# xu-ji/IIC

Measured on AMD Instinct MI355X. Metric: paired-images/sec, STL10 96x96 ClusterNet5g+IID_loss, higher is better.
Workload: dtype bf16; 1 GPU; STL10 96x96 ClusterNet5g IID+ (cluster_sobel.py train step), batch 660 pairs/GPU, 5 sub-heads, k=70, bf16 MFMA convs / fp32 stem+heads+loss, fused HIP Adam; global_batch_pairs=660, input=96x96x1 grey -> sobel 2ch, parallelism=dp1, streams=2, launch=hip-graph replay: 6 linear graph segments, the two views on two streams

## Files before the change

iic_amd/csrc/common.h:

```cpp
#pragma once
#include <hip/hip_runtime.h>
#include <stdint.h>

#include <atomic>
#include <mutex>
#include <utility>

#define IIC_OK 0
#define IIC_ERR_ARG (-1)
#define IIC_ERR_LAUNCH (-2)
#define IIC_ERR_UNSUPPORTED (-3)

#ifdef IIC_DEBUG_HOOKS
#define IIC_HOOK extern "C" __attribute__((visibility("default")))
#define IIC_SWITCH(var, dflt, setter) \
  static int var = dflt;              \
  IIC_HOOK void setter(int v) { var = v; }
IIC_HOOK int iic_debug_get_ablate(void);
#else
#define IIC_SWITCH(var, dflt, setter) static constexpr int var = dflt;
static inline constexpr int iic_debug_get_ablate(void) { return 0; }
#endif

typedef __attribute__((ext_vector_type(8))) __bf16 bf16x8;
typedef __attribute__((ext_vector_type(4))) short s16x4;
typedef __attribute__((ext_vector_type(16))) float f32x16;
typedef __attribute__((ext_vector_type(4))) float f32x4;
typedef __attribute__((ext_vector_type(4))) unsigned int u32x4;
typedef __attribute__((ext_vector_type(2))) unsigned int u32x2;

typedef uint16_t bf16_t;

static inline int iic_launch_status() {
  hipError_t e = hipGetLastError();
  return e == hipSuccess ? IIC_OK : IIC_ERR_LAUNCH;
}

static constexpr long IIC_LDS_BYTES = 160 * 1024;

template <auto Kernel, typename... Args>
inline int iic_launch_lds(dim3 grid, dim3 block, size_t lds, hipStream_t s, Args&&... args) {
  static std::atomic<size_t> limit{48 * 1024};
  if (lds > limit.load(std::memory_order_acquire)) {
    static std::mutex raise;
// ... 128 lines not shown
```

iic_amd/csrc/conv_igemm_bd.hip:

```cpp
#include "common.h"
#include "conv_tile.h"
#include "../../include/iic_hip.h"

__device__ __forceinline__ void bd_bload(u32x4& d, const unsigned char* p) {
  asm volatile("global_load_dwordx4 %0, %1, off" : "=v"(d) : "v"(p) : "memory");
}
template <int N>
__device__ __forceinline__ void bd_bwait(u32x4& d) {
  asm volatile("s_waitcnt vmcnt(%1)" : "+v"(d) : "i"(N) : "memory");
}

struct bd_blk {
  int bw, bh, nbx, nby;
  int PW, npix, mul;
};

#define BD_BM 256
#define BD_BN 128
#define BD_THREADS 256
#define BD_PROF_SLOTS 16
#ifndef BD_STORE_UB
#define BD_STORE_UB 8
#endif

template <bool GATHER, int ABL, int MS, int RED, int WN = 2>
__device__ __forceinline__ void bd_tile(
    const iic_conv_geom& g, const bf16_t* __restrict__ in, const unsigned char* __restrict__ wfrag,
    bf16_t* __restrict__ out, float* __restrict__ stats, const bf16_t* __restrict__ res_grad,
    const bf16_t* __restrict__ res_act, int accumulate, int lds_a_bytes,
    const bf16_t* __restrict__ red_y, const float* __restrict__ red_coef,
    const bf16_t* __restrict__ red_y2, float* __restrict__ red_stats, float* __restrict__ red_stats2,
    unsigned long long* __restrict__ prof, int blk_in_class, int nwg_class, const bd_blk& B) {
  constexpr int BNT = WN * 64, NWM = 4 / WN;
  constexpr bool CANBLK = !GATHER && MS * 32 * (4 / WN) == 256;
  const bool blk = CANBLK && B.bw > 0;
  constexpr int CLD = BNT + 8;
  constexpr bool PROF = (ABL & 128) != 0;
  constexpr bool NEWORD = (ABL & 256) == 0;
  constexpr bool SWZ = (ABL & 512) == 0;
  unsigned long long t_stamp[8];
  unsigned long long t_bsum = 0, t_b0 = 0;
  int t_nb = 0;
  if (PROF) t_stamp[0] = __builtin_readcyclecounter();
  constexpr int BM = MS * 32 * NWM, WR = MS * 32;
  extern __shared__ __attribute__((aligned(16))) unsigned char smem_raw[];
  unsigned char* sA = smem_raw;
  int* s_pin = reinterpret_cast<int*>(smem_raw + lds_a_bytes);
  int* s_pout = s_pin + BM;
  float* s_red = reinterpret_cast<float*>(s_pout + BM);
  unsigned char* s_key = reinterpret_cast<unsigned char*>(s_red + NWM * 2 * BNT);
  bf16_t* sC = reinterpret_cast<bf16_t*>(smem_raw);

  const int tid = threadIdx.x, lane = tid & 63;
  const int wave = __builtin_amdgcn_readfirstlane(tid >> 6);
  const int wm = WN == 2 ? wave >> 1 : wave, wn = WN == 2 ? wave & 1 : 0;
  const int l31 = lane & 31, g5 = lane >> 5;

  const int nt = g.Cout / BNT;
  const int tix = xcd_tile_index(blk_in_class, nwg_class);
  const int mtile = tix / nt, ntile = tix - mtile * nt;
  const int n0 = ntile * BNT;
  const int m0 = mtile * BM;
// ... 22 lines not shown
    }
  } else if (tid < BM) {
    int pin, pout;
    igemm_row_pixels(g, m0 + tid, pin, pout);
    s_pin[tid] = pin;
    s_pout[tid] = pout;
  }
  __syncthreads();
  const int p_lo = blk ? 0 : s_pin[0];
  const int npix = GATHER ? BM : (blk ? B.npix : (BM >= 192 ? g.NP256 : g.NP));
  const int keyw = blk ? B.PW : g.in_Wp;
  const int jskip = blk ? B.PW - B.bw
                        : ((!GATHER && g.sx == 1 && ((g.in_Wp - g.MX) & 1) == 0) ? g.in_Wp - g.MX : 0);
  auto dense_of = [&](int p) { return p - jskip * (p / keyw); };
  int arow[MS];
  int drow[MS];
#pragma unroll
  for (int ms = 0; ms < MS; ++ms) {
    const int row = wm * WR + ms * 32 + l31;
    const int pr = GATHER ? row : (s_pin[row] - p_lo);
    arow[ms] = SWZ ? pr : pr * ROWB + g5 * 16;
    drow[ms] = (SWZ && !GATHER) ? dense_of(s_pin[row]) : pr;
  }
  if (!GATHER && jskip != 0) {
    for (int r = tid; r < npix; r += BD_THREADS) s_key[r] = (unsigned char)((dense_of(p_lo + r) >> 1) & 7);
    __syncthreads();
  }
  const int v_tapd = v_tapoff - jskip * (v_tapoff / keyw);
  const int nblk = (npix * 128 + 1023) >> 10;
  auto dma_patch = [&](int c0) {
    for (int kb = wave; kb < nblk; kb += BD_THREADS / 64) {
      const int q = kb * 64 + lane;
      const int r = q >> 3;
      const int ls = (q & 7) ^ (GATHER ? ((r >> 1) & 7)
                                       : (jskip != 0 ? (int)s_key[r < npix ? r : npix - 1]
                                                     : (((p_lo + r) >> 1) & 7)));
      long p = GATHER ? (long)s_pin[r < BM ? r : BM - 1] : (long)p_lo + r;
      if (blk) {
        const int rc = r < npix ? r : npix - 1;
        const int py = (rc * B.mul) >> 16;
        p = (long)blk_glo + py * g.in_Wp + (rc - py * B.PW);
      }
      p = p < in_pixels ? p : in_pixels - 1;
      __builtin_amdgcn_global_load_lds(
          (const __attribute__((address_space(1))) void*)(in + (p * g.Cin + c0 + ls * 8)),
          (__attribute__((address_space(3))) void*)(sA + kb * 1024), 16, 0, 0);
    }
    asm volatile("s_waitcnt vmcnt(0)" ::: "memory");
  };
  auto a_base = [&](int R, int D) { return R * 128 + (((g5 ^ (D >> 1)) & 1) << 4); };
  auto a_kk = [&](int D) { return ((D >> 2) & 3) << 5; };

  f32x16 acc[MS][2];
// ... 208 lines not shown
      }
  __syncthreads();
  if (PROF) t_stamp[4] = __builtin_readcyclecounter();
  TileRed tr;
  if (RED) tile_red_zero(tr);
  if (!(ABL & 32))
    igemm_store_tile<BNT, BM, BD_THREADS, 8, RED, (BM == 256 ? BD_STORE_UB : 4)>(sC, s_pout, out, res_grad, res_act, accumulate,
                                                                 g.Cout, n0, tid, red_y, red_coef, red_y2, &tr);
  if (RED)
    igemm_red_finish<BNT, BD_THREADS, RED>(tr, reinterpret_cast<float*>(smem_raw), red_stats, red_stats2,
                                             g.Cout, n0, tid);
  if (PROF && prof && tid == 0) {
    unsigned long long* q = prof + (long)blockIdx.x * BD_PROF_SLOTS;
    const unsigned long long t_end = __builtin_readcyclecounter();
    q[0] = t_stamp[0]; q[1] = t_stamp[1]; q[2] = t_stamp[2]; q[3] = t_stamp[3]; q[4] = t_stamp[4];
    q[5] = t_end; q[6] = t_bsum; q[7] = (unsigned long long)t_nb;
    q[8] = (unsigned long long)__builtin_amdgcn_s_getreg((32 - 1) << 11 | 0 << 6 | 4)
           | ((unsigned long long)__builtin_amdgcn_s_getreg((4 - 1) << 11 | 0 << 6 | 20) << 32);
    q[9] = (unsigned long long)tix;
    q[10] = __builtin_amdgcn_s_memrealtime();
  }
}

template <bool GATHER, int ABL, int MS, int RED, int WN = 2>
__global__ __launch_bounds__(BD_THREADS, ((MS == 4 || WN == 1) ? 2 : 3)) void conv_igemm_bd_kernel(
    const iic_conv_geom g, const bf16_t* __restrict__ in, const unsigned char* __restrict__ wfrag,
    bf16_t* __restrict__ out, float* __restrict__ stats, const bf16_t* __restrict__ res_grad,
    const bf16_t* __restrict__ res_act, int accumulate, int num_mtiles, int lds_a_bytes,
    const bf16_t* __restrict__ red_y, const float* __restrict__ red_coef,
    const bf16_t* __restrict__ red_y2, float* __restrict__ red_stats, float* __restrict__ red_stats2,
    unsigned long long* __restrict__ prof, const bd_blk B) {
  bd_tile<GATHER, ABL, MS, RED, WN>(g, in, wfrag, out, stats, res_grad, res_act, accumulate, lds_a_bytes, red_y,
                                    red_coef, red_y2, red_stats, red_stats2, prof, (int)blockIdx.x,
                                    num_mtiles * (g.Cout / (WN * 64)), B);
}

__global__ void weight_prep_frag_kernel(const float* __restrict__ w, bf16_t* __restrict__ o, int Co,
                                        int Ci, int T, int mode) {
  const int Nn = mode ? Ci : Co, Kk = mode ? Co : Ci;
  const int n32 = Nn >> 5, nchunks = Kk >> 6;
  const long total = (long)T * Co * Ci;
  for (long i = (long)blockIdx.x * blockDim.x + threadIdx.x; i < total;
       i += (long)gridDim.x * blockDim.x) {
    const int e = (int)(i & 7), lane = (int)((i >> 3) & 63), ks = (int)((i >> 9) & 3);
    long r = i >> 11;
    const int j = (int)(r % n32);
    r /= n32;
    const int kc = (int)(r % nchunks), t = (int)(r / nchunks);
    const int n = j * 32 + (lane & 31), k = kc * 64 + ks * 16 + (lane >> 5) * 8 + e;
    const int co = mode ? k : n, ci = mode ? n : k;
    o[i] = f32_to_bf16(w[((long)co * Ci + ci) * T + t]);
  }
}

int iic_p64_supported(const iic_conv_geom* g);
int iic_p64_launch(const iic_conv_geom* g, const void* in, const void* wfrag, void* out, float* stats,
                   const void* res_grad, const void* res_act, int accumulate, const void* red_y,
                   const float* red_coef, const void* red_y2, float* red_stats, float* red_stats2,
                   void* stream);
int iic_pw_supported(const iic_conv_geom* g);
int iic_pw_launch(const iic_conv_geom* g, const void* in, const void* wfrag, void* out, float* stats,
                  const void* res_grad, const void* res_act, int accumulate, const void* red_y,
                  const float* red_coef, const void* red_y2, float* red_stats, float* red_stats2, void* stream);
IIC_SWITCH(g_p64_enabled, 1, iic_debug_enable_p64)
IIC_SWITCH(g_p64_red, 0, iic_debug_p64_red)

extern "C" {

#ifdef IIC_DEBUG_HOOKS
static unsigned long long* g_bd_prof = nullptr;
IIC_HOOK void iic_debug_bd_prof(void* buf) { g_bd_prof = (unsigned long long*)buf; }
IIC_HOOK int iic_debug_bd_prof_slots(void) { return BD_PROF_SLOTS; }
#else
static constexpr unsigned long long* g_bd_prof = nullptr;
#endif

static long bd_lds_a(const iic_conv_geom* g, int ms, int wn = 2) {
  const long bm = ms * 32 * (4 / wn);
  const long npix = g->ntaps == 1 ? bm : (bm >= 192 ? g->NP256 : g->NP);
  long a = (npix * 128 + 1023) & ~1023L;
  long c = bm * (wn * 64 + 8) * 2;
  long m = a > c ? a : c;
  return (m + 15) & ~15L;
}

static long bd_key_bytes(const iic_conv_geom* g, int ms, int wn = 2) {
  const int jskip = (g->ntaps > 1 && g->sx == 1 && ((g->in_Wp - g->MX) & 1) == 0) ? g->in_Wp - g->MX : 0;
  return jskip != 0 ? (((long)(ms * 32 * (4 / wn) >= 192 ? g->NP256 : g->NP) + 15) & ~15L) : 0;
}
static long bd_lds_total(const iic_conv_geom* g, int ms, int wn = 2) {
  return bd_lds_a(g, ms, wn) + 2L * ms * 32 * (4 / wn) * 4 + 4L * BD_BN * 4 + bd_key_bytes(g, ms, wn);
}
IIC_SWITCH(g_bd_w1, 1, iic_debug_bd_w1)
static bool bd_w1_ok(const iic_conv_geom* g) {
  return g_bd_w1 && g->Cout % 64 == 0 && g->Cout % BD_BN != 0 && g->ntaps > 1 && g->NP256 > 0 &&
         bd_lds_total(g, 2, 1) <= IIC_LDS_BYTES;
}
IIC_SWITCH(g_bd_ms, 0, iic_debug_bd_ms)
static int bd_pick_ms(const iic_conv_geom* g) {
  const bool ok4 = (g->ntaps == 1 || g->NP256 > 0) && bd_lds_total(g, 4) <= IIC_LDS_BYTES;
  const bool ok2 = (g->ntaps == 1 || g->NP > 0) && bd_lds_total(g, 2) <= IIC_LDS_BYTES;
  if (g_bd_ms == 4) return ok4 ? 4 : (ok2 ? 2 : 0);
  if (g_bd_ms == 2) return ok2 ? 2 : (ok4 ? 4 : 0);
  if (ok4 && ok2 && g->ntaps > 1) {
    const long M = igemm_rows_host(g);
    if (((M + 255) / 256) * (g->Cout / BD_BN) * 2 <= 512) return 2;
  }
  return ok4 ? 4 : (ok2 ? 2 : 0);
}

static int bd_block_config(const iic_conv_geom* g, bd_blk* B, int wn);
int iic_conv_igemm_frag_supported(const iic_conv_geom* g) {
  if (!g) return 0;
  if (g_p64_enabled && iic_p64_supported(g)) return 1;
// ... 93 lines not shown
      const long a = ((long)B1.npix * 128 + 1023) & ~1023L, c = (long)BD_BM * (64 + 8) * 2;
      la1 = (int)(((a > c ? a : c) + 15) & ~15L);
      lds1 = la1 + 2L * BD_BM * 4 + 4L * BD_BN * 4 + ((B1.npix + 15) & ~15L);
    }
    hipStream_t s1 = (hipStream_t)stream;
    int rc1 = IIC_OK;
#define BD_LAUNCH_W1(RD_)                                                                              \
  rc1 = iic_launch_lds<conv_igemm_bd_kernel<false, 0, 2, RD_, 1>>(                                     \
      dim3(grid1), dim3(BD_THREADS), lds1, s1, *g, (const bf16_t*)in, (const unsigned char*)wfrag,     \
      (bf16_t*)out, stats, (const bf16_t*)res_grad, (const bf16_t*)res_act, accumulate, mt1, la1,      \
      (const bf16_t*)red_y, red_coef, (const bf16_t*)red_y2, red_stats, red_stats2,                    \
      (unsigned long long*)nullptr, B1)
    if (red == 0) BD_LAUNCH_W1(0); else if (red == 1) BD_LAUNCH_W1(1); else BD_LAUNCH_W1(2);
    return rc1 ? rc1 : iic_launch_status();
  }
  bd_blk BB = {0, 0, 0, 0, 0, 0, 0};
  const bool blocked = iic_debug_get_ablate() == 0 && bd_block_config(g, &BB, 2) != 0;
  const int ms = blocked ? 4 : bd_pick_ms(g);
  if (ms == 0) return IIC_ERR_UNSUPPORTED;
  const int bm = ms * 64;
  const int mt = blocked ? g->N * BB.nbx * BB.nby : (int)((M + bm - 1) / bm);
  const int nt = g->Cout / BD_BN;
  const int grid = mt * nt;
  int la = (int)bd_lds_a(g, ms);
  long lds = bd_lds_total(g, ms);
  if (blocked) {
    const long a = ((long)BB.npix * 128 + 1023) & ~1023L, c = (long)BD_BM * (BD_BN + 8) * 2;
    la = (int)(((a > c ? a : c) + 15) & ~15L);
    lds = la + 2L * BD_BM * 4 + 4L * BD_BN * 4 + ((BB.npix + 15) & ~15L);
  }
  hipStream_t s = (hipStream_t)stream;
  int rc = IIC_OK;
#define BD_LAUNCH4(GA_, AB_, MS_, RD_)                                                            \
  rc = iic_launch_lds<conv_igemm_bd_kernel<GA_, AB_, MS_, RD_>>(                                 \
      dim3(grid), dim3(BD_THREADS), lds, s, *g, (const bf16_t*)in, (const unsigned char*)wfrag,  \
      (bf16_t*)out, stats, (const bf16_t*)res_grad, (const bf16_t*)res_act, accumulate, mt, la,  \
      (const bf16_t*)red_y, red_coef, (const bf16_t*)red_y2, red_stats, red_stats2, g_bd_prof, BB)
#define BD_LAUNCH3(GA_, AB_, MS_)                                                                 \
  do {                                                                                           \
    if ((AB_ != 0 && AB_ != 128 && AB_ != 256) || GA_ || red == 0) {                             \
      if (red != 0) return IIC_ERR_UNSUPPORTED;                                                  \
      BD_LAUNCH4(GA_, AB_, MS_, 0);                                                              \
    } else if (red == 1) BD_LAUNCH4(false, (AB_ == 128 || AB_ == 256 ? AB_ : 0), MS_, 1);        \
    else BD_LAUNCH4(false, (AB_ == 128 || AB_ == 256 ? AB_ : 0), MS_, 2);                        \
  } while (0)
#define BD_LAUNCH(GA_, AB_)                                                                       \
  do {                                                                                           \
    if (ms == 4) BD_LAUNCH3(GA_, AB_, 4); else BD_LAUNCH3(GA_, AB_, 2);                          \
  } while (0)
  if (g->ntaps == 1) BD_LAUNCH(true, 0);
  else switch (iic_debug_get_ablate()) {
#ifdef IIC_BD_ABLATIONS
    case 1: BD_LAUNCH(false, 1); break;
    case 2: BD_LAUNCH(false, 2); break;
    case 3: BD_LAUNCH(false, 3); break;
    case 4: BD_LAUNCH(false, 4); break;
    case 7: BD_LAUNCH(false, 7); break;
    case 15: BD_LAUNCH(false, 15); break;
    case 16: BD_LAUNCH(false, 16); break;
    case 31: BD_LAUNCH(false, 31); break;
    case 32: BD_LAUNCH(false, 32); break;
    case 64: BD_LAUNCH(false, 64); break;
    case 96: BD_LAUNCH(false, 96); break;
    case 128: BD_LAUNCH(false, 128); break;
    case 256: BD_LAUNCH(false, 256); break;
    case 512: BD_LAUNCH(false, 512); break;
#endif
    default: BD_LAUNCH(false, 0); break;
  }
  return rc ? rc : iic_launch_status();
}

__global__ __launch_bounds__(256) void weight_prep_multi_kernel(const iic_weight_prep_job* __restrict__ jobs,
                                                                int njobs) {
  int lo = 0, hi = njobs - 1;
  while (lo < hi) {
    const int mid = (lo + hi + 1) >> 1;
    if ((long long)blockIdx.x >= jobs[mid].first_block) lo = mid; else hi = mid - 1;
  }
  const iic_weight_prep_job j = jobs[lo];
  const float* __restrict__ w = j.w;
  bf16_t* __restrict__ o = reinterpret_cast<bf16_t*>(j.out);
  const int Co = j.Cout, Ci = j.Cin, T = j.T, mode = j.mode;
  const long total = (long)T * Co * Ci;
  const long nblk = (total + 2047) >> 11;
  const long b = (long)blockIdx.x - j.first_block;
  if (b >= nblk) return;
  for (long i = b * 256 + threadIdx.x; i < total; i += nblk * 256) {
    if (mode <= 1) {
      const int Nn = mode ? Ci : Co, Kk = mode ? Co : Ci;
      const int n32 = Nn >> 5, nchunks = Kk >> 6;
      const int e = (int)(i & 7), lane = (int)((i >> 3) & 63), ks = (int)((i >> 9) & 3);
      long r = i >> 11;
      const int jj = (int)(r % n32);
// ... 43 lines not shown
```

iic_amd/csrc/conv_igemm_pw.hip:

```cpp
#include <type_traits>

#include "common.h"
#include "conv_tile.h"
#include "../../include/iic_hip.h"

#define PW_THREADS 256
#define PW_STG_LD 72
#define PW_STG_BYTES (32 * PW_STG_LD * 2)
#define PW_KEYS 512
#define PW_PROF_SLOTS 32

struct pw_div {
  unsigned mul;
  int sh;
};
static inline pw_div pw_make_div(int d) {
  pw_div r;
  int l = 0;
  while ((1L << l) < d) ++l;
  r.sh = 31 + l;
  r.mul = (unsigned)(((1ULL << r.sh) + (unsigned long long)d - 1) / (unsigned long long)d);
  if (d == 1) { r.mul = 1u << 31; r.sh = 31; }
  return r;
}
__device__ __forceinline__ int pw_divide(int n, const pw_div& d) {
  return (int)(((unsigned long long)(unsigned)n * d.mul) >> d.sh);
}

struct pw_args {
  pw_div d_rows;
  pw_div d_mx;
  pw_div d_wp;
  int rows_per_img;
  int plane;
  int jskip;
  int npix;
  int patch_bytes;
  int mt;
  int M;
  int in_pixels;
  int pad_rows;
};

template <int OFF>
__device__ __forceinline__ void pw_bload(u32x4& d, unsigned voff, const unsigned char* sbase) {
  asm volatile("global_load_dwordx4 %0, %1, %2 offset:%3" : "=v"(d) : "v"(voff), "s"(sbase), "n"(OFF) : "memory");
}
template <int N>
__device__ __forceinline__ void pw_bwait(u32x4& d) {
  asm volatile("s_waitcnt vmcnt(%1)" : "+v"(d) : "n"(N) : "memory");
}
__device__ __forceinline__ void pw_dma16(const void* gsrc, unsigned lds_dst) {
  unsigned keep;
  asm volatile(
      "s_mov_b32 %0, m0\n\ts_mov_b32 m0, %2\n\ts_nop 0\n\tglobal_load_lds_dwordx4 %1, off\n\ts_mov_b32 m0, %0"
      : "=&s"(keep)
      : "v"(gsrc), "s"(lds_dst)
      : "memory");
}

__device__ __forceinline__ void pw_row(const iic_conv_geom& g, const pw_args& A, int m, int& pin, int& prow,
                                       int& pout) {
  int n = pw_divide(m, A.d_rows);
  int r = m - n * A.rows_per_img;
  const bool valid = n < g.N && r < A.plane;
  if (n >= g.N) { n = g.N - 1; r = A.plane - 1; }
  r = r < A.plane ? r : A.plane - 1;
  const int y = pw_divide(r, A.d_mx), x = r - y * g.MX;
  prow = n * g.in_Hp + y * g.sy + g.oy;
  pin = prow * g.in_Wp + x * g.sx + g.ox;
  pout = valid ? (n * g.out_Hp + y * g.ty + g.py) * g.out_Wp + x * g.tx + g.px : -1;
}
template <int RED, int U>
__device__ __forceinline__ void pw_store_pass(const bf16_t* sW, int u0, const int (&po)[4], bf16_t* __restrict__ out,
                                               const bf16_t* __restrict__ res_grad, const bf16_t* __restrict__ res_act,
                                               int accumulate, int Cout, int col0, int lane,
                                               const bf16_t* __restrict__ red_y, bool red_mask,
                                               const float (&msc)[8], const float (&msh)[8],
                                               const bf16_t* __restrict__ red_y2, TileRed& red) {
  const bool add_prev = accumulate & IIC_ACC_ADD, premask = accumulate & IIC_ACC_PREMASK;
// ... 62 lines not shown
      for (int i = 0; i < 4; ++i) {
        gq[2 * i] = bf16lo(gq4[i]); gq[2 * i + 1] = bf16hi(gq4[i]);
        yq[2 * i] = bf16lo(yy[i]); yq[2 * i + 1] = bf16hi(yy[i]);
      }
      if (red_mask) {
#pragma unroll
        for (int i = 0; i < 8; ++i)
          if (!(yq[i] * msc[i] + msh[i] > 0.f)) gq[i] = 0.f;
      }
#pragma unroll
      for (int i = 0; i < 8; ++i) { red.s[i] += gq[i]; red.sy[i] += gq[i] * yq[i]; }
      if (RED == 2) {
        const uint32_t zz[4] = {zv[u].x, zv[u].y, zv[u].z, zv[u].w};
#pragma unroll
        for (int i = 0; i < 4; ++i) {
          red.sy2[2 * i] += gq[2 * i] * bf16lo(zz[i]);
          red.sy2[2 * i + 1] += gq[2 * i + 1] * bf16hi(zz[i]);
        }
      }
    }
  }
}

template <int RED, bool PROF>
__global__ __launch_bounds__(PW_THREADS, 2) void conv_igemm_pw_kernel(
    const iic_conv_geom g, const pw_args A, const bf16_t* __restrict__ in, const unsigned char* __restrict__ wfrag,
    bf16_t* __restrict__ out, float* __restrict__ stats, const bf16_t* __restrict__ res_grad,
    const bf16_t* __restrict__ res_act, int accumulate, const bf16_t* __restrict__ red_y,
    const float* __restrict__ red_coef, const bf16_t* __restrict__ red_y2, float* __restrict__ red_stats,
    float* __restrict__ red_stats2, unsigned long long* __restrict__ prof) {
  extern __shared__ __attribute__((aligned(16))) unsigned char smem_raw[];
  const int tid = threadIdx.x, lane = tid & 63;
  const int wave = __builtin_amdgcn_readfirstlane(tid >> 6);
  const int wm = wave >> 1, wn = wave & 1;
  const int l31 = lane & 31, g5 = lane >> 5;
  unsigned char* sA = smem_raw;
  bf16_t* sW = reinterpret_cast<bf16_t*>(smem_raw + A.patch_bytes + wave * PW_STG_BYTES);
  unsigned char* s_key = smem_raw + A.patch_bytes + 4 * PW_STG_BYTES;
  const unsigned lds0 = (unsigned)(size_t)(__attribute__((address_space(3))) unsigned char*)sA;

  unsigned long long t_all = 0, t_wait = 0, t_k = 0, t_b = 0, t_e = 0, t0 = 0, t1 = 0;
  int n_tiles = 0, n_b = 0;
  unsigned long long t_line[4][4];
  unsigned long long rt0 = 0;
  if (PROF) {
    rt0 = __builtin_amdgcn_s_memrealtime();
    t_all = __builtin_readcyclecounter();
#pragma unroll
    for (int i = 0; i < 4; ++i)
#pragma unroll
      for (int j = 0; j < 4; ++j) t_line[i][j] = 0;
  }

  const int nt = g.Cout >> 7;
  const int xcd = blockIdx.x & 7, kx = blockIdx.x >> 3, Gx = gridDim.x >> 3;
  const int ntile = xcd & (nt - 1), per = 8 / nt, xr = xcd / nt;
  const int mt_lo = (int)((long)A.mt * xr / per), mt_hi = (int)((long)A.mt * (xr + 1) / per);
  const int n0 = ntile << 7;
  int mtile = mt_lo + kx;
  if (mtile >= mt_hi) return;

  const int v_tapoff = g.tap_off[lane & (IIC_MAX_TAPS - 1)];
  const int v_tapw = g.tap_w[lane & (IIC_MAX_TAPS - 1)];
  const int v_tapd = v_tapoff - A.jskip * pw_divide(v_tapoff, A.d_wp);
  const int nchunks = g.Cin >> 6, ntaps = g.ntaps, NIT = nchunks * ntaps;
  const int nblk = A.patch_bytes >> 10;
  const long frag_it = (long)(g.Cout >> 5) * 4096;
  const unsigned boff = (unsigned)(((n0 + wn * 64) >> 5) * 4096 + lane * 16);
  auto frag_base = [&](int tap, int chunk) {
    const int tw = __builtin_amdgcn_readlane(v_tapw, tap);
    return wfrag + ((long)tw * nchunks + chunk) * frag_it + 4096;
  };

  auto tile_plo = [&](int mtl) {
    int pin, prow, pout;
    pw_row(g, A, mtl << 8, pin, prow, pout);
    return __builtin_amdgcn_readfirstlane(pin);
  };
  auto write_keys = [&](int p_lo_t, int kb) {
    for (int r = tid; r < PW_KEYS; r += PW_THREADS) {
      const int p = p_lo_t + r;
      const int prow = pw_divide(p, A.d_wp);
      const int D = p - A.jskip * prow;
      const int key = (D >> 1) & 7;
      s_key[kb * PW_KEYS + r] = (unsigned char)key;
    }
  };
  auto dma_patch = [&](int p_lo_t, int c0, int kb) {
    for (int blk = wave; blk < nblk; blk += PW_THREADS / 64) {
      const int q = blk * 64 + lane;
      const int r = q >> 3;
      const int ls = (q & 7) ^ ((int)s_key[kb * PW_KEYS + r] & 7);
      long p = (long)p_lo_t + r;
      p = p < A.in_pixels ? p : A.in_pixels - 1;
      pw_dma16(in + (p * g.Cin + c0 + ls * 8),
               (unsigned)__builtin_amdgcn_readfirstlane((int)(lds0 + (unsigned)(blk * 1024))));
    }
  };

  float st_s[2] = {0.f, 0.f}, st_ss[2] = {0.f, 0.f};
  TileRed tr;
  tile_red_zero(tr);
  const bool red_mask = RED && red_coef != nullptr;

  int kb = 0;
  int p_lo = tile_plo(mtile);
  write_keys(p_lo, 0);
  __syncthreads();
  dma_patch(p_lo, 0, 0);

  for (;;) {
    const int m0 = mtile << 8;
    const int mnext = mtile + Gx;
    const bool has_next = mnext < mt_hi;
    if (PROF) {
      t0 = __builtin_readcyclecounter();
#pragma unroll
      for (int i = 0; i < 4; ++i) if (n_tiles == i) t_line[i][0] = t0;
    }

    int arow[4], drow[4];
#pragma unroll
    for (int ms = 0; ms < 4; ++ms) {
      int pin, prow, pout;
      pw_row(g, A, m0 + wm * 128 + ms * 32 + l31, pin, prow, pout);
      arow[ms] = pin - p_lo;
      drow[ms] = pin - A.jskip * prow;
    }
    int p_lo_next = 0;
    if (has_next) {
      p_lo_next = tile_plo(mnext);
      write_keys(p_lo_next, kb ^ 1);
    }
    auto tap_p = [&](int ms, int toff, int td) {
      const int R = arow[ms] + toff, D = drow[ms] + td;
      return (R << 7) + ((((D >> 1) ^ g5) & 1) << 4);
    };
    auto tap_k = [&](int ms, int td) { return (((drow[ms] + td) >> 2) & 3) << 5; };

    f32x16 acc[4][2];
#pragma unroll
    for (int ms = 0; ms < 4; ++ms)
#pragma unroll
      for (int ns = 0; ns < 2; ++ns)
#pragma unroll
        for (int r = 0; r < 16; ++r) acc[ms][ns][r] = 0.f;

    u32x4 Bc[4][2];
    {
      const unsigned char* sb = frag_base(0, 0);
      pw_bload<-4096>(Bc[0][0], boff, sb); pw_bload<0>(Bc[0][1], boff, sb);
      pw_bload<-3072>(Bc[1][0], boff, sb); pw_bload<1024>(Bc[1][1], boff, sb);
      pw_bload<-2048>(Bc[2][0], boff, sb); pw_bload<2048>(Bc[2][1], boff, sb);
      pw_bload<-1024>(Bc[3][0], boff, sb); pw_bload<3072>(Bc[3][1], boff, sb);
    }
    asm volatile("s_waitcnt vmcnt(8)\n\ts_waitcnt lgkmcnt(0)" ::: "memory");
    __builtin_amdgcn_s_barrier();
    if (PROF) {
      t1 = __builtin_readcyclecounter(); t_wait += t1 - t0; t0 = t1;
#pragma unroll
      for (int i = 0; i < 4; ++i) if (n_tiles == i) t_line[i][1] = t1;
    }

    int pa[2][4], ka[2][4];
    bf16x8 a[2][4];
    auto lds16 = [](int addr) {
      return *reinterpret_cast<const __attribute__((address_space(3))) bf16x8*>((size_t)(unsigned)addr);
    };
    {
      const int toff = __builtin_amdgcn_readlane(v_tapoff, 0), td = __builtin_amdgcn_readlane(v_tapd, 0);
#pragma unroll
      for (int ms = 0; ms < 4; ++ms) {
        pa[0][ms] = (int)lds0 + tap_p(ms, toff, td);
        ka[0][ms] = tap_k(ms, td);
        a[0][ms] = lds16(pa[0][ms] + ka[0][ms]);
      }
    }

    int tap_n = 0, chunk_n = 0;
    bool more_n = false, bnd_n = false;
    const unsigned char* nb = nullptr;
    int toffn = 0, tdn = 0;
    auto advance = [&](int t, int c, int& t2, int& c2, bool& more2, bool& bnd2) {
      t2 = t + 1; c2 = c;
      if (t2 == ntaps) { t2 = 0; ++c2; }
      more2 = c2 < nchunks;
      bnd2 = more2 && t2 == 0;
      if (!more2) { t2 = t; c2 = c; }
    };
    advance(0, 0, tap_n, chunk_n, more_n, bnd_n);
    nb = frag_base(tap_n, chunk_n);
    toffn = __builtin_amdgcn_readlane(v_tapoff, tap_n);
    tdn = __builtin_amdgcn_readlane(v_tapd, tap_n);
    auto body = [&](auto parsel) {
      constexpr int P = decltype(parsel)::value, Q = P ^ 1;
      int tap_2 = 0, chunk_2 = 0, toff2 = 0, td2 = 0;
      bool more_2 = false, bnd_2 = false;
      const unsigned char* nb2 = nullptr;
#pragma unroll
      for (int ks = 0; ks < 4; ++ks) {
        const int cur = ks & 1, nxt = cur ^ 1;
        pw_bwait<7>(Bc[ks][0]);
        __builtin_amdgcn_sched_barrier(0);
        const bf16x8 b0 = __builtin_bit_cast(bf16x8, Bc[ks][0]);
#pragma unroll
        for (int ms = 0; ms < 4; ++ms) {
          acc[ms][0] = __builtin_amdgcn_mfma_f32_32x32x16_bf16(a[cur][ms], b0, acc[ms][0], 0, 0, 0);
          a[nxt][ms] = (ks < 3) ? lds16(pa[P][ms] + (((ks + 1) << 5) ^ ka[P][ms])) : lds16(pa[Q][ms] + ka[Q][ms]);
          __builtin_amdgcn_sched_barrier(0);
        }
        pw_bwait<6>(Bc[ks][1]);
        if (ks == 0) pw_bload<-4096>(Bc[0][0], boff, nb);
        if (ks == 1) pw_bload<-3072>(Bc[1][0], boff, nb);
        if (ks == 2) pw_bload<-2048>(Bc[2][0], boff, nb);
        if (ks == 3) pw_bload<-1024>(Bc[3][0], boff, nb);
        __builtin_amdgcn_sched_barrier(0);
        const bf16x8 b1 = __builtin_bit_cast(bf16x8, Bc[ks][1]);
#pragma unroll
        for (int ms = 0; ms < 4; ++ms) {
          acc[ms][1] = __builtin_amdgcn_mfma_f32_32x32x16_bf16(a[cur][ms], b1, acc[ms][1], 0, 0, 0);
          if (ks == 0) pa[Q][ms] = (int)lds0 + tap_p(ms, toffn, tdn);
          if (ks == 1) ka[Q][ms] = tap_k(ms, tdn);
          if (ks == 2 && ms == 0) advance(tap_n, chunk_n, tap_2, chunk_2, more_2, bnd_2);
          if (ks == 2 && ms == 1) nb2 = frag_base(tap_2, chunk_2);
          if (ks == 2 && ms == 2) {
            toff2 = __builtin_amdgcn_readlane(v_tapoff, tap_2);
            td2 = __builtin_amdgcn_readlane(v_tapd, tap_2);
          }
          __builtin_amdgcn_sched_barrier(0);
        }
        if (ks == 0) pw_bload<0>(Bc[0][1], boff, nb);
        if (ks == 1) pw_bload<1024>(Bc[1][1], boff, nb);
        if (ks == 2) pw_bload<2048>(Bc[2][1], boff, nb);
        if (ks == 3) pw_bload<3072>(Bc[3][1], boff, nb);
        __builtin_amdgcn_sched_barrier(0);
      }
      if (bnd_n) {
        if (PROF) t1 = __builtin_readcyclecounter();
        asm volatile("s_waitcnt lgkmcnt(0)" ::: "memory");
        __builtin_amdgcn_s_barrier();
        dma_patch(p_lo, chunk_n * 64, kb);
        asm volatile("s_waitcnt vmcnt(0)" ::: "memory");
        __builtin_amdgcn_s_barrier();
        if (PROF) { t_b += __builtin_readcyclecounter() - t1; ++n_b; }
// ... 129 lines not shown
        if (RED == 2) {
          iic_stat_add(red_stats2, stripe, g.Cout, col, 0, tr.s[i]);
          iic_stat_add(red_stats2, stripe, g.Cout, col, 1, tr.sy2[i]);
        }
      }
    }
  }
  if (PROF && prof && tid == 0) {
    unsigned long long* q = prof + (long)blockIdx.x * PW_PROF_SLOTS;
    q[0] = t_wait; q[1] = t_k; q[2] = t_b; q[3] = t_e;
    q[4] = __builtin_readcyclecounter() - t_all;
    q[5] = (unsigned long long)n_tiles; q[6] = (unsigned long long)n_b;
#pragma unroll
    for (int i = 0; i < 4; ++i)
#pragma unroll
      for (int j = 0; j < 4; ++j) q[8 + i * 4 + j] = t_line[i][j];
    q[24] = rt0;
    q[25] = __builtin_amdgcn_s_memrealtime();
    q[7] = (unsigned long long)__builtin_amdgcn_s_getreg((32 - 1) << 11 | 0 << 6 | 4) | ((unsigned long long)__builtin_amdgcn_s_getreg((4 - 1) << 11 | 0 << 6 | 20) << 32);
  }
}

IIC_SWITCH(g_pw_enabled, 1, iic_debug_enable_pw)
#ifdef IIC_DEBUG_HOOKS
static unsigned long long* g_pw_prof = nullptr;
IIC_HOOK void iic_debug_pw_prof(void* buf) { g_pw_prof = (unsigned long long*)buf; }
IIC_HOOK int iic_debug_pw_prof_slots(void) { return PW_PROF_SLOTS; }
IIC_HOOK int iic_debug_pw_grid(const iic_conv_geom* g);
#else
static constexpr unsigned long long* g_pw_prof = nullptr;
#endif

static long pw_lds_bytes(const iic_conv_geom* g) {
  const long patch = ((long)g->NP256 * 128 + 1023) & ~1023L;
  return patch + 4 * PW_STG_BYTES + 2 * PW_KEYS;
}

static int pw_num_cus();
static int pw_supported_shape(const iic_conv_geom* g);
int iic_pw_supported(const iic_conv_geom* g) {
  if (!g || !g_pw_enabled || !pw_supported_shape(g)) return 0;
  const long M = igemm_rows_host(g);
  if (((M + 255) / 256) * (g->Cout / 128) * 10 < 25L * 2 * pw_num_cus()) return 0;
  return 1;
}
static int pw_supported_shape(const iic_conv_geom* g) {
  if (!g) return 0;
  if (g->ntaps < 2 || g->ntaps > IIC_MAX_TAPS || g->Cin % 64 != 0 || g->Cout % 128 != 0) return 0;
  const int nt = g->Cout / 128;
  if (nt != 1 && nt != 2 && nt != 4 && nt != 8) return 0;
  if (g->NP256 <= 0 || g->NP256 > PW_KEYS) return 0;
  if (pw_lds_bytes(g) > 80 * 1024) return 0;
  const long M = igemm_rows_host(g);
  if (M <= 0 || M + 256 >= (1L << 31) || (long)g->N * g->in_Hp * g->in_Wp >= (1L << 31)) return 0;
  return 1;
}

static int pw_num_cus() {
  static int n = 0;
  if (n == 0) {
    int dev = 0;
    hipDeviceProp_t prop;
    if (hipGetDevice(&dev) == hipSuccess && hipGetDeviceProperties(&prop, dev) == hipSuccess) n = prop.multiProcessorCount;
    if (n <= 0) n = 256;
  }
  return n;
}

static int pw_grid(const iic_conv_geom* g, long lds) {
  const long M = igemm_rows_host(g);
  const int mt = (int)((M + 255) / 256), nt = g->Cout / 128, per = 8 / nt;
  int longest = 0;
  for (int xr = 0; xr < per; ++xr) {
    const int len = (int)((long)mt * (xr + 1) / per) - (int)((long)mt * xr / per);
    longest = len > longest ? len : longest;
  }
  const int slots = (lds <= 80 * 1024 ? 2 : 1) * pw_num_cus();
  int gx = slots / 8;
  if (gx > longest) gx = longest;
  if (gx < 1) gx = 1;
  return gx * 8;
}
#ifdef IIC_DEBUG_HOOKS
IIC_HOOK int iic_debug_pw_grid(const iic_conv_geom* g) { return g ? pw_grid(g, pw_lds_bytes(g)) : 0; }
#endif

int iic_pw_launch(const iic_conv_geom* g, const void* in, const void* wfrag, void* out, float* stats,
                  const void* res_grad, const void* res_act, int accumulate, const void* red_y,
                  const float* red_coef, const void* red_y2, float* red_stats, float* red_stats2, void* stream) {
  if (!iic_pw_supported(g)) return IIC_ERR_UNSUPPORTED;
  const long M = igemm_rows_host(g);
  pw_args A;
  A.plane = g->MY * g->MX;
  A.rows_per_img = g->MP > 0 ? g->MP : A.plane;
  A.d_rows = pw_make_div(A.rows_per_img);
  A.d_mx = pw_make_div(g->MX);
  A.d_wp = pw_make_div(g->in_Wp);
  A.jskip = (g->sx == 1 && ((g->in_Wp - g->MX) & 1) == 0) ? g->in_Wp - g->MX : 0;
  A.npix = g->NP256;
  A.patch_bytes = (int)(((long)g->NP256 * 128 + 1023) & ~1023L);
  A.mt = (int)((M + 255) / 256);
  A.M = (int)M;
  A.in_pixels = g->N * g->in_Hp * g->in_Wp;
  A.pad_rows = (g->MP > 0 && g->MP != A.plane) ? 1 : 0;
  const long lds = pw_lds_bytes(g);
  const int grid = pw_grid(g, lds);
  const int red = red_y ? (red_y2 ? 2 : 1) : 0;
  hipStream_t s = (hipStream_t)stream;
  int rc = IIC_OK;
#define PW_LAUNCH(RD_, PR_)                                                                                   \
  rc = iic_launch_lds<conv_igemm_pw_kernel<RD_, PR_>>(                                                        \
      dim3(grid), dim3(PW_THREADS), lds, s, *g, A, (const bf16_t*)in, (const unsigned char*)wfrag,            \
      (bf16_t*)out, stats, (const bf16_t*)res_grad, (const bf16_t*)res_act, accumulate, (const bf16_t*)red_y, \
      red_coef, (const bf16_t*)red_y2, red_stats, red_stats2, g_pw_prof)
#ifdef IIC_DEBUG_HOOKS
  if (g_pw_prof) {
    if (red == 0) PW_LAUNCH(0, true); else if (red == 1) PW_LAUNCH(1, true); else PW_LAUNCH(2, true);
    return rc ? rc : iic_launch_status();
  }
#endif
  if (red == 0) PW_LAUNCH(0, false); else if (red == 1) PW_LAUNCH(1, false); else PW_LAUNCH(2, false);
  return rc ? rc : iic_launch_status();
}
```

iic_amd/csrc/conv_tile.h:

```cpp
#pragma once
#include "common.h"
#include "../../include/iic_hip.h"

__device__ __forceinline__ void igemm_row_pixels(const iic_conv_geom& g, int m, int& pin, int& pout) {
  const int plane = g.MY * g.MX;
  const int mp = g.MP > 0 ? g.MP : plane;
  int n = m / mp;
  int r = m - n * mp;
  const bool valid = n < g.N && r < plane;
  if (n >= g.N) { n = g.N - 1; r = plane - 1; }
  r = r < plane ? r : plane - 1;
  const int y = r / g.MX, x = r - y * g.MX;
  pin = (n * g.in_Hp + y * g.sy + g.oy) * g.in_Wp + x * g.sx + g.ox;
  pout = valid ? (n * g.out_Hp + y * g.ty + g.py) * g.out_Wp + x * g.tx + g.px : -1;
}
__device__ __forceinline__ int igemm_rows(const iic_conv_geom& g) {
  return g.N * (g.MP > 0 ? g.MP : g.MY * g.MX);
}
__device__ __forceinline__ bool igemm_tile_has_invalid(const iic_conv_geom& g, int m0, int bm) {
  const int plane = g.MY * g.MX;
  if (m0 + bm > igemm_rows(g)) return true;
  return g.MP > 0 && g.MP != plane && (m0 % g.MP) + bm > plane;
}
static inline long igemm_rows_host(const iic_conv_geom* g) {
  return (long)g->N * (g->MP > 0 ? g->MP : g->MY * g->MX);
}
static inline bool igemm_dense_host(const iic_conv_geom* g) { return g->MP <= 0 || g->MP == g->MY * g->MX; }

#define ROWB 144

__device__ __forceinline__ int xcd_tile_index(int b, int nwg) {
  const int q = nwg >> 3, r = nwg & 7, xcd = b & 7, idx = b >> 3;
  return (xcd < r ? xcd * (q + 1) : r * (q + 1) + (xcd - r) * q) + idx;
}

template <bool GATHER, int NTHREADS, int NB = 4>
__device__ __forceinline__ void igemm_load_patch(unsigned char* sA, const bf16_t* __restrict__ in,
                                                 int Cin, int c0, int p_lo, int npix,
                                                 int in_pixels, const int* s_pin, int tid) {
  const int n8 = npix * 8;
  for (int base = 0; base < n8; base += NTHREADS * NB) {
    u32x4 v[NB];
#pragma unroll
    for (int u = 0; u < NB; ++u) {
      const int idx = base + u * NTHREADS + tid;
      v[u] = (u32x4){0u, 0u, 0u, 0u};
      if (idx < n8) {
        const long p = GATHER ? (long)s_pin[idx >> 3] : (long)p_lo + (idx >> 3);
        if (p < in_pixels) v[u] = *reinterpret_cast<const u32x4*>(in + (p * Cin + c0 + (idx & 7) * 8));
      }
    }
#pragma unroll
// ... 171 lines not shown
```

Measured before the change: 18880 paired-images/sec.

## Stage conv input patches in LDS with padded 144-byte row pitch

Adds a padded LDS patch layout (144-byte rows, 7 rows per 1008-byte piece, written with global_load_lds) for the multi-tap bd and pw implicit-GEMM conv kernels. It replaces the XOR swizzle and key tables, so bank conflicts are avoided by the pitch instead and the per-tap key/jskip address arithmetic goes away. In exchange the patch buffer grows and some DMA lanes are wasted (9 lanes per row, one duplicated), which may reduce occupancy. The new path is gated by LDS caps and enabled by default. It also drops the ABL 512 debug variant and adds grid-cap and pw-enable debug switches.

```diff
diff --git a/iic_amd/csrc/common.h b/iic_amd/csrc/common.h
--- a/iic_amd/csrc/common.h
+++ b/iic_amd/csrc/common.h
@@ -11,15 +11,18 @@
 #define IIC_ERR_LAUNCH (-2)
 #define IIC_ERR_UNSUPPORTED (-3)
 
+#define IIC_BD_PITCH144 1
 #ifdef IIC_DEBUG_HOOKS
 #define IIC_HOOK extern "C" __attribute__((visibility("default")))
 #define IIC_SWITCH(var, dflt, setter) \
   static int var = dflt;              \
   IIC_HOOK void setter(int v) { var = v; }
 IIC_HOOK int iic_debug_get_ablate(void);
+IIC_HOOK int iic_debug_get_bd_pitch144(void);
 #else
 #define IIC_SWITCH(var, dflt, setter) static constexpr int var = dflt;
 static inline constexpr int iic_debug_get_ablate(void) { return 0; }
+static inline constexpr int iic_debug_get_bd_pitch144(void) { return IIC_BD_PITCH144; }
 #endif
 
 typedef __attribute__((ext_vector_type(8))) __bf16 bf16x8;
diff --git a/iic_amd/csrc/conv_igemm_bd.hip b/iic_amd/csrc/conv_igemm_bd.hip
--- a/iic_amd/csrc/conv_igemm_bd.hip
+++ b/iic_amd/csrc/conv_igemm_bd.hip
@@ -23,7 +23,7 @@
 #define BD_STORE_UB 8
 #endif
 
-template <bool GATHER, int ABL, int MS, int RED, int WN = 2>
+template <bool GATHER, int ABL, int MS, int RED, int WN = 2, bool PAD = false>
 __device__ __forceinline__ void bd_tile(
     const iic_conv_geom& g, const bf16_t* __restrict__ in, const unsigned char* __restrict__ wfrag,
     bf16_t* __restrict__ out, float* __restrict__ stats, const bf16_t* __restrict__ res_grad,
@@ -33,11 +33,12 @@
     unsigned long long* __restrict__ prof, int blk_in_class, int nwg_class, const bd_blk& B) {
   constexpr int BNT = WN * 64, NWM = 4 / WN;
   constexpr bool CANBLK = !GATHER && MS * 32 * (4 / WN) == 256;
-  const bool blk = CANBLK && B.bw > 0;
+  const bool blk = CANBLK && !PAD && B.bw > 0;
   constexpr int CLD = BNT + 8;
   constexpr bool PROF = (ABL & 128) != 0;
   constexpr bool NEWORD = (ABL & 256) == 0;
-  constexpr bool SWZ = (ABL & 512) == 0;
+  static_assert(!(PAD && GATHER), "the padded patch is a multi-tap form");
+  constexpr bool SWZ = !PAD;
   unsigned long long t_stamp[8];
   unsigned long long t_bsum = 0, t_b0 = 0;
   int t_nb = 0;
@@ -106,13 +107,26 @@
     arow[ms] = SWZ ? pr : pr * ROWB + g5 * 16;
     drow[ms] = (SWZ && !GATHER) ? dense_of(s_pin[row]) : pr;
   }
-  if (!GATHER && jskip != 0) {
+  if (SWZ && !GATHER && jskip != 0) {
     for (int r = tid; r < npix; r += BD_THREADS) s_key[r] = (unsigned char)((dense_of(p_lo + r) >> 1) & 7);
     __syncthreads();
   }
   const int v_tapd = v_tapoff - jskip * (v_tapoff / keyw);
   const int nblk = (npix * 128 + 1023) >> 10;
+  const int dma_rl = lane / 9, dma_pc = min(lane - dma_rl * 9, 7) * 8;
   auto dma_patch = [&](int c0) {
+    if (PAD) {
+      const int nj = (npix + PT144_ROWS - 1) / PT144_ROWS;
+      for (int j = wave; j < nj; j += BD_THREADS / 64) {
+        long p = (long)p_lo + j * PT144_ROWS + dma_rl;
+        p = p < in_pixels ? p : in_pixels - 1;
+        __builtin_amdgcn_global_load_lds(
+            (const __attribute__((address_space(1))) void*)(in + (p * g.Cin + c0 + dma_pc)),
+            (__attribute__((address_space(3))) void*)(sA + j * PT144_PIECE), 16, 0, 0);
+      }
+      asm volatile("s_waitcnt vmcnt(0)" ::: "memory");
+      return;
+    }
     for (int kb = wave; kb < nblk; kb += BD_THREADS / 64) {
       const int q = kb * 64 + lane;
       const int r = q >> 3;
@@ -367,7 +381,7 @@
   }
 }
 
-template <bool GATHER, int ABL, int MS, int RED, int WN = 2>
+template <bool GATHER, int ABL, int MS, int RED, int WN = 2, bool PAD = false>
 __global__ __launch_bounds__(BD_THREADS, ((MS == 4 || WN == 1) ? 2 : 3)) void conv_igemm_bd_kernel(
     const iic_conv_geom g, const bf16_t* __restrict__ in, const unsigned char* __restrict__ wfrag,
     bf16_t* __restrict__ out, float* __restrict__ stats, const bf16_t* __restrict__ res_grad,
@@ -375,7 +389,7 @@
     const bf16_t* __restrict__ red_y, const float* __restrict__ red_coef,
     const bf16_t* __restrict__ red_y2, float* __restrict__ red_stats, float* __restrict__ red_stats2,
     unsigned long long* __restrict__ prof, const bd_blk B) {
-  bd_tile<GATHER, ABL, MS, RED, WN>(g, in, wfrag, out, stats, res_grad, res_act, accumulate, lds_a_bytes, red_y,
+  bd_tile<GATHER, ABL, MS, RED, WN, PAD>(g, in, wfrag, out, stats, res_grad, res_act, accumulate, lds_a_bytes, red_y,
                                     red_coef, red_y2, red_stats, red_stats2, prof, (int)blockIdx.x,
                                     num_mtiles * (g.Cout / (WN * 64)), B);
 }
@@ -420,10 +434,10 @@
 static constexpr unsigned long long* g_bd_prof = nullptr;
 #endif
 
-static long bd_lds_a(const iic_conv_geom* g, int ms, int wn = 2) {
+static long bd_lds_a(const iic_conv_geom* g, int ms, int wn = 2, bool pad = false) {
   const long bm = ms * 32 * (4 / wn);
   const long npix = g->ntaps == 1 ? bm : (bm >= 192 ? g->NP256 : g->NP);
-  long a = (npix * 128 + 1023) & ~1023L;
+  long a = pad ? pt144_bytes(npix) : (npix * 128 + 1023) & ~1023L;
   long c = bm * (wn * 64 + 8) * 2;
   long m = a > c ? a : c;
   return (m + 15) & ~15L;
@@ -433,8 +447,17 @@
   const int jskip = (g->ntaps > 1 && g->sx == 1 && ((g->in_Wp - g->MX) & 1) == 0) ? g->in_Wp - g->MX : 0;
   return jskip != 0 ? (((long)(ms * 32 * (4 / wn) >= 192 ? g->NP256 : g->NP) + 15) & ~15L) : 0;
 }
-static long bd_lds_total(const iic_conv_geom* g, int ms, int wn = 2) {
-  return bd_lds_a(g, ms, wn) + 2L * ms * 32 * (4 / wn) * 4 + 4L * BD_BN * 4 + bd_key_bytes(g, ms, wn);
+static long bd_lds_total(const iic_conv_geom* g, int ms, int wn = 2, bool pad = false) {
+  return bd_lds_a(g, ms, wn, pad) + 2L * ms * 32 * (4 / wn) * 4 + 4L * BD_BN * 4 + (pad ? 0 : bd_key_bytes(g, ms, wn));
+}
+IIC_SWITCH(g_bd_pitch144, IIC_BD_PITCH144, iic_debug_bd_pitch144)
+#ifdef IIC_DEBUG_HOOKS
+IIC_HOOK int iic_debug_get_bd_pitch144(void) { return g_bd_pitch144; }
+#endif
+static bool bd_pad_ok(const iic_conv_geom* g, int ms) {
+  if (!g_bd_pitch144 || g->ntaps < 2 || g->sx != 1 || g->sy != 1) return false;
+  const long cap = ms == 4 ? 80 * 1024 : 160 * 1024 / 3;
+  return bd_lds_total(g, ms, 2, true) <= cap;
 }
 IIC_SWITCH(g_bd_w1, 1, iic_debug_bd_w1)
 static bool bd_w1_ok(const iic_conv_geom* g) {
@@ -574,8 +597,9 @@
   const int mt = blocked ? g->N * BB.nbx * BB.nby : (int)((M + bm - 1) / bm);
   const int nt = g->Cout / BD_BN;
   const int grid = mt * nt;
-  int la = (int)bd_lds_a(g, ms);
-  long lds = bd_lds_total(g, ms);
+  const bool pad = !blocked && iic_debug_get_ablate() == 0 && bd_pad_ok(g, ms);
+  int la = (int)bd_lds_a(g, ms, 2, pad);
+  long lds = bd_lds_total(g, ms, 2, pad);
   if (blocked) {
     const long a = ((long)BB.npix * 128 + 1023) & ~1023L, c = (long)BD_BM * (BD_BN + 8) * 2;
     la = (int)(((a > c ? a : c) + 15) & ~15L);
@@ -583,11 +607,16 @@
   }
   hipStream_t s = (hipStream_t)stream;
   int rc = IIC_OK;
-#define BD_LAUNCH4(GA_, AB_, MS_, RD_)                                                            \
-  rc = iic_launch_lds<conv_igemm_bd_kernel<GA_, AB_, MS_, RD_>>(                                 \
+#define BD_LAUNCH5(GA_, AB_, MS_, RD_, PD_)                                                       \
+  rc = iic_launch_lds<conv_igemm_bd_kernel<GA_, AB_, MS_, RD_, 2, PD_>>(                         \
       dim3(grid), dim3(BD_THREADS), lds, s, *g, (const bf16_t*)in, (const unsigned char*)wfrag,  \
       (bf16_t*)out, stats, (const bf16_t*)res_grad, (const bf16_t*)res_act, accumulate, mt, la,  \
       (const bf16_t*)red_y, red_coef, (const bf16_t*)red_y2, red_stats, red_stats2, g_bd_prof, BB)
+#define BD_LAUNCH4(GA_, AB_, MS_, RD_)                                                            \
+  do {                                                                                           \
+    if (!GA_ && AB_ == 0 && pad) BD_LAUNCH5(false, 0, MS_, RD_, true);                           \
+    else BD_LAUNCH5(GA_, AB_, MS_, RD_, false);                                                  \
+  } while (0)
 #define BD_LAUNCH3(GA_, AB_, MS_)                                                                 \
   do {                                                                                           \
     if ((AB_ != 0 && AB_ != 128 && AB_ != 256) || GA_ || red == 0) {                             \
@@ -616,12 +645,23 @@
     case 96: BD_LAUNCH(false, 96); break;
     case 128: BD_LAUNCH(false, 128); break;
     case 256: BD_LAUNCH(false, 256); break;
-    case 512: BD_LAUNCH(false, 512); break;
 #endif
     default: BD_LAUNCH(false, 0); break;
   }
   return rc ? rc : iic_launch_status();
 }
+
+#ifdef IIC_DEBUG_HOOKS
+IIC_HOOK int iic_debug_pw_pitch144_used(const iic_conv_geom* g);
+IIC_HOOK int iic_debug_bd_pitch144_used(const iic_conv_geom* g) {
+  if (!g || !iic_conv_igemm_frag_supported(g) || (g_p64_enabled && iic_p64_supported(g))) return 0;
+  if (iic_debug_get_ablate() == 0 && g_bd_ms == 0 && iic_pw_supported(g)) return iic_debug_pw_pitch144_used(g) ? 2 : 0;
+  bd_blk B;
+  if (g->Cout % BD_BN != 0 || iic_debug_get_ablate() != 0 || bd_block_config(g, &B, 2)) return 0;
+  const int ms = bd_pick_ms(g);
+  return ms != 0 && bd_pad_ok(g, ms) ? 1 : 0;
+}
+#endif
 
 __global__ __launch_bounds__(256) void weight_prep_multi_kernel(const iic_weight_prep_job* __restrict__ jobs,
                                                                 int njobs) {
diff --git a/iic_amd/csrc/conv_igemm_pw.hip b/iic_amd/csrc/conv_igemm_pw.hip
--- a/iic_amd/csrc/conv_igemm_pw.hip
+++ b/iic_amd/csrc/conv_igemm_pw.hip
@@ -40,6 +40,7 @@
   int M;
   int in_pixels;
   int pad_rows;
+  int nj;
 };
 
 template <int OFF>
@@ -56,6 +57,15 @@
       "s_mov_b32 %0, m0\n\ts_mov_b32 m0, %2\n\ts_nop 0\n\tglobal_load_lds_dwordx4 %1, off\n\ts_mov_b32 m0, %0"
       : "=&s"(keep)
       : "v"(gsrc), "s"(lds_dst)
+      : "memory");
+}
+
+__device__ __forceinline__ void pw_dma16s(unsigned voff, const unsigned char* sbase, unsigned lds_dst) {
+  unsigned keep;
+  asm volatile(
+      "s_mov_b32 %0, m0\n\ts_mov_b32 m0, %3\n\ts_nop 0\n\tglobal_load_lds_dwordx4 %1, %2\n\ts_mov_b32 m0, %0"
+      : "=&s"(keep)
+      : "v"(voff), "s"(sbase), "s"(lds_dst)
       : "memory");
 }
 
@@ -164,7 +174,7 @@
   }
 }
 
-template <int RED, bool PROF>
+template <int RED, bool PROF, bool PAD>
 __global__ __launch_bounds__(PW_THREADS, 2) void conv_igemm_pw_kernel(
     const iic_conv_geom g, const pw_args A, const bf16_t* __restrict__ in, const unsigned char* __restrict__ wfrag,
     bf16_t* __restrict__ out, float* __restrict__ stats, const bf16_t* __restrict__ res_grad,
@@ -202,9 +212,9 @@
   int mtile = mt_lo + kx;
   if (mtile >= mt_hi) return;
 
-  const int v_tapoff = g.tap_off[lane & (IIC_MAX_TAPS - 1)];
+  const int v_tapoff = g.tap_off[lane & (IIC_MAX_TAPS - 1)] * (PAD ? ROWB : 1);
   const int v_tapw = g.tap_w[lane & (IIC_MAX_TAPS - 1)];
-  const int v_tapd = v_tapoff - A.jskip * pw_divide(v_tapoff, A.d_wp);
+  const int v_tapd = PAD ? 0 : v_tapoff - A.jskip * pw_divide(v_tapoff, A.d_wp);
   const int nchunks = g.Cin >> 6, ntaps = g.ntaps, NIT = nchunks * ntaps;
   const int nblk = A.patch_bytes >> 10;
   const long frag_it = (long)(g.Cout >> 5) * 4096;
@@ -220,6 +230,7 @@
     return __builtin_amdgcn_readfirstlane(pin);
   };
   auto write_keys = [&](int p_lo_t, int kb) {
+    if (PAD) return;
     for (int r = tid; r < PW_KEYS; r += PW_THREADS) {
       const int p = p_lo_t + r;
       const int prow = pw_divide(p, A.d_wp);
@@ -228,7 +239,21 @@
       s_key[kb * PW_KEYS + r] = (unsigned char)key;
     }
   };
+  const int dma_rl = lane / 9;
+  const unsigned dma_pc = (unsigned)min(lane - dma_rl * 9, 7) * 16u;
+  const unsigned dma_voff = (unsigned)(dma_rl * g.Cin * 2) + dma_pc;
   auto dma_patch = [&](int p_lo_t, int c0, int kb) {
+    if (PAD) {
+      const unsigned char* tb = reinterpret_cast<const unsigned char*>(in + ((long)p_lo_t * g.Cin + c0));
+      const int rmax = A.in_pixels - 1 - p_lo_t, rowb = g.Cin * 2;
+      for (int j = wave; j < A.nj; j += PW_THREADS / 64) {
+        const int r0 = j * PT144_ROWS;
+        const unsigned dst = (unsigned)__builtin_amdgcn_readfirstlane((int)(lds0 + (unsigned)(j * PT144_PIECE)));
+        if (r0 + PT144_ROWS <= rmax) pw_dma16s(dma_voff, tb + (long)r0 * rowb, dst);
+        else pw_dma16s((unsigned)(min(r0 + dma_rl, rmax) * rowb) + dma_pc, tb, dst);
+      }
+      return;
+    }
     for (int blk = wave; blk < nblk; blk += PW_THREADS / 64) {
       const int q = blk * 64 + lane;
       const int r = q >> 3;
@@ -266,8 +291,8 @@
     for (int ms = 0; ms < 4; ++ms) {
       int pin, prow, pout;
       pw_row(g, A, m0 + wm * 128 + ms * 32 + l31, pin, prow, pout);
-      arow[ms] = pin - p_lo;
-      drow[ms] = pin - A.jskip * prow;
+      arow[ms] = PAD ? (int)lds0 + (pin - p_lo) * ROWB + g5 * 16 : pin - p_lo;
+      drow[ms] = PAD ? 0 : pin - A.jskip * prow;
     }
     int p_lo_next = 0;
     if (has_next) {
@@ -275,10 +300,11 @@
       write_keys(p_lo_next, kb ^ 1);
     }
     auto tap_p = [&](int ms, int toff, int td) {
+      if (PAD) return arow[ms] + toff;
       const int R = arow[ms] + toff, D = drow[ms] + td;
-      return (R << 7) + ((((D >> 1) ^ g5) & 1) << 4);
+      return (int)lds0 + (R << 7) + ((((D >> 1) ^ g5) & 1) << 4);
     };
-    auto tap_k = [&](int ms, int td) { return (((drow[ms] + td) >> 2) & 3) << 5; };
+    auto tap_k = [&](int ms, int td) { return PAD ? 0 : (((drow[ms] + td) >> 2) & 3) << 5; };
 
     f32x16 acc[4][2];
 #pragma unroll
@@ -313,7 +339,7 @@
       const int toff = __builtin_amdgcn_readlane(v_tapoff, 0), td = __builtin_amdgcn_readlane(v_tapd, 0);
 #pragma unroll
       for (int ms = 0; ms < 4; ++ms) {
-        pa[0][ms] = (int)lds0 + tap_p(ms, toff, td);
+        pa[0][ms] = tap_p(ms, toff, td);
         ka[0][ms] = tap_k(ms, td);
         a[0][ms] = lds16(pa[0][ms] + ka[0][ms]);
       }
@@ -348,7 +374,8 @@
 #pragma unroll
         for (int ms = 0; ms < 4; ++ms) {
           acc[ms][0] = __builtin_amdgcn_mfma_f32_32x32x16_bf16(a[cur][ms], b0, acc[ms][0], 0, 0, 0);
-          a[nxt][ms] = (ks < 3) ? lds16(pa[P][ms] + (((ks + 1) << 5) ^ ka[P][ms])) : lds16(pa[Q][ms] + ka[Q][ms]);
+          if (PAD) a[nxt][ms] = (ks < 3) ? lds16(pa[P][ms] + ((ks + 1) << 5)) : lds16(pa[Q][ms]);
+          else a[nxt][ms] = (ks < 3) ? lds16(pa[P][ms] + (((ks + 1) << 5) ^ ka[P][ms])) : lds16(pa[Q][ms] + ka[Q][ms]);
           __builtin_amdgcn_sched_barrier(0);
         }
         pw_bwait<6>(Bc[ks][1]);
@@ -361,7 +388,7 @@
 #pragma unroll
         for (int ms = 0; ms < 4; ++ms) {
           acc[ms][1] = __builtin_amdgcn_mfma_f32_32x32x16_bf16(a[cur][ms], b1, acc[ms][1], 0, 0, 0);
-          if (ks == 0) pa[Q][ms] = (int)lds0 + tap_p(ms, toffn, tdn);
+          if (ks == 0) pa[Q][ms] = tap_p(ms, toffn, tdn);
           if (ks == 1) ka[Q][ms] = tap_k(ms, tdn);
           if (ks == 2 && ms == 0) advance(tap_n, chunk_n, tap_2, chunk_2, more_2, bnd_2);
           if (ks == 2 && ms == 1) nb2 = frag_base(tap_2, chunk_2);
@@ -537,6 +564,7 @@
 }
 
 IIC_SWITCH(g_pw_enabled, 1, iic_debug_enable_pw)
+IIC_SWITCH(g_pw_gx_cap, 0, iic_debug_pw_gx_cap)
 #ifdef IIC_DEBUG_HOOKS
 static unsigned long long* g_pw_prof = nullptr;
 IIC_HOOK void iic_debug_pw_prof(void* buf) { g_pw_prof = (unsigned long long*)buf; }
@@ -546,9 +574,13 @@
 static constexpr unsigned long long* g_pw_prof = nullptr;
 #endif
 
-static long pw_lds_bytes(const iic_conv_geom* g) {
+static long pw_lds_bytes(const iic_conv_geom* g, bool pad = false) {
+  if (pad) return pt144_bytes(g->NP256) + 4 * PW_STG_BYTES;
   const long patch = ((long)g->NP256 * 128 + 1023) & ~1023L;
   return patch + 4 * PW_STG_BYTES + 2 * PW_KEYS;
+}
+static bool pw_pad_ok(const iic_conv_geom* g) {
+  return iic_debug_get_bd_pitch144() != 0 && g->sx == 1 && g->sy == 1 && pw_lds_bytes(g, true) <= 80 * 1024;
 }
 
 static int pw_num_cus();
@@ -556,7 +588,7 @@
 int iic_pw_supported(const iic_conv_geom* g) {
   if (!g || !g_pw_enabled || !pw_supported_shape(g)) return 0;
   const long M = igemm_rows_host(g);
-  if (((M + 255) / 256) * (g->Cout / 128) * 10 < 25L * 2 * pw_num_cus()) return 0;
+  if (g_pw_enabled != 2 && ((M + 255) / 256) * (g->Cout / 128) * 10 < 25L * 2 * pw_num_cus()) return 0;
   return 1;
 }
 static int pw_supported_shape(const iic_conv_geom* g) {
@@ -593,11 +625,13 @@
   const int slots = (lds <= 80 * 1024 ? 2 : 1) * pw_num_cus();
   int gx = slots / 8;
   if (gx > longest) gx = longest;
+  if (g_pw_gx_cap > 0 && gx > g_pw_gx_cap) gx = g_pw_gx_cap;
   if (gx < 1) gx = 1;
   return gx * 8;
 }
 #ifdef IIC_DEBUG_HOOKS
 IIC_HOOK int iic_debug_pw_grid(const iic_conv_geom* g) { return g ? pw_grid(g, pw_lds_bytes(g)) : 0; }
+IIC_HOOK int iic_debug_pw_pitch144_used(const iic_conv_geom* g) { return g && iic_pw_supported(g) && pw_pad_ok(g) ? 1 : 0; }
 #endif
 
 int iic_pw_launch(const iic_conv_geom* g, const void* in, const void* wfrag, void* out, float* stats,
@@ -618,16 +652,23 @@
   A.M = (int)M;
   A.in_pixels = g->N * g->in_Hp * g->in_Wp;
   A.pad_rows = (g->MP > 0 && g->MP != A.plane) ? 1 : 0;
-  const long lds = pw_lds_bytes(g);
+  const bool pad = pw_pad_ok(g);
+  A.nj = (int)((g->NP256 + PT144_ROWS - 1) / PT144_ROWS);
+  if (pad) A.patch_bytes = (int)pt144_bytes(g->NP256);
+  const long lds = pw_lds_bytes(g, pad);
   const int grid = pw_grid(g, lds);
   const int red = red_y ? (red_y2 ? 2 : 1) : 0;
   hipStream_t s = (hipStream_t)stream;
   int rc = IIC_OK;
-#define PW_LAUNCH(RD_, PR_)                                                                                   \
-  rc = iic_launch_lds<conv_igemm_pw_kernel<RD_, PR_>>(                                                        \
+#define PW_LAUNCH2(RD_, PR_, PD_)                                                                             \
+  rc = iic_launch_lds<conv_igemm_pw_kernel<RD_, PR_, PD_>>(                                                   \
       dim3(grid), dim3(PW_THREADS), lds, s, *g, A, (const bf16_t*)in, (const unsigned char*)wfrag,            \
       (bf16_t*)out, stats, (const bf16_t*)res_grad, (const bf16_t*)res_act, accumulate, (const bf16_t*)red_y, \
       red_coef, (const bf16_t*)red_y2, red_stats, red_stats2, g_pw_prof)
+#define PW_LAUNCH(RD_, PR_)                                                                                   \
+  do {                                                                                                        \
+    if (pad) PW_LAUNCH2(RD_, PR_, true); else PW_LAUNCH2(RD_, PR_, false);                                    \
+  } while (0)
 #ifdef IIC_DEBUG_HOOKS
   if (g_pw_prof) {
     if (red == 0) PW_LAUNCH(0, true); else if (red == 1) PW_LAUNCH(1, true); else PW_LAUNCH(2, true);
diff --git a/iic_amd/csrc/conv_tile.h b/iic_amd/csrc/conv_tile.h
--- a/iic_amd/csrc/conv_tile.h
+++ b/iic_amd/csrc/conv_tile.h
@@ -28,6 +28,11 @@
 static inline bool igemm_dense_host(const iic_conv_geom* g) { return g->MP <= 0 || g->MP == g->MY * g->MX; }
 
 #define ROWB 144
+#define PT144_ROWS 7
+#define PT144_PIECE (PT144_ROWS * ROWB)
+static inline long pt144_bytes(long npix) {
+  return ((npix + PT144_ROWS - 1) / PT144_ROWS) * PT144_PIECE + 16;
+}
 
 __device__ __forceinline__ int xcd_tile_index(int b, int nwg) {
   const int q = nwg >> 3, r = nwg & 7, xcd = b & 7, idx = b >> 3;
```

Measured after the change: 19350 paired-images/sec (median of 6 runs). +2.5%, better.
